# panthuncia/BasicRenderer

Measured on AMD Instinct MI355X. Metric: shaded Mpixels/s @4K (vis-buffer+resolve), higher is better.
Workload: dtype f32; 1 GPU; bistro-class procedural frame, 3840x2160, 1 directional + 256 point lights, 22669824 instanced tris, 2017 instances (2614016 in 150 meshes), LOD DAGs from the library's cluster-LOD builder, relief slope 1.5; pixels_per_gpu=8294400, visible_clusters_rank0=10118, occlusion_culling=True, visible_clusters_phase2_rank0=0, meshlets_tested_rank0=26713, partition=single GPU, frames_in_flight=3

## Files before the change

### basicrenderer_amd/capi.py

```python
import ctypes as C
import os

_HERE = os.path.dirname(os.path.abspath(__file__))
LIB_DIR = os.path.join(_HERE, "lib")

u32, u64, f32, vp = C.c_uint32, C.c_uint64, C.c_float, C.c_void_p


class SceneParams(C.Structure):
    _fields_ = [("preset", u32), ("seed", u32), ("width", u32), ("height", u32), ("numPointLights", u32),
                ("withDirectionalLight", u32), ("lodLevels", u32), ("sizeScale", f32), ("skinnedFraction1024", u32),
                ("materialFeatures", u32), ("cameraStep", u32), ("lodBuilder", u32), ("spotLightEvery", u32), ("detail", f32), ("uniqueTriangleBudget", u32), ("reliefSlope", f32)]


class MeshInput(C.Structure):
    _fields_ = [("positions", vp), ("normals", vp), ("uvs", vp), ("colors", vp), ("vertexCount", C.c_size_t), ("indices", vp), ("indexCount", C.c_size_t),
                ("material", u32), ("reserved", u32 * 3)]


class InstanceInput(C.Structure):
    _fields_ = [("mesh", u32), ("reverseWinding", u32), ("model", (f32 * 4) * 4)]


class ViewInput(C.Structure):
# ... 265 lines not shown
        lib.brmi_scene_export_cache.argtypes = [vp, C.c_char_p]
        lib.brmi_scene_destroy.argtypes = [vp]
        lib.brmi_scene_array.argtypes = [vp, u32, C.POINTER(vp), C.POINTER(u64), C.POINTER(u32)]
        lib.brmi_scene_slab_count.argtypes = [vp]
        lib.brmi_scene_slab_count.restype = u32
        lib.brmi_scene_slab.argtypes = [vp, u32, C.POINTER(vp), C.POINTER(u64)]
        lib.brmi_scene_get_stats.argtypes = [vp, C.POINTER(SceneStats)]
        lib.brmi_scene_camera_at.argtypes = [C.POINTER(SceneParams), C.c_double, C.c_double, vp, vp]
        _scene_lib = lib
    return _scene_lib


BRMI_EXPORTS = ["brmi_abi_version", "brmi_default_config", "brmi_create", "brmi_declare", "brmi_set_scene", "brmi_setup", "brmi_set_band",
                "brmi_update", "brmi_execute", "brmi_execute_split", "brmi_destroy", "brmi_last_error", "brmi_clear_visibility", "brmi_cull",
                "brmi_raster", "brmi_depth_copy", "brmi_build_hzb", "brmi_invalidate_hzb", "brmi_set_history_source", "brmi_gbuffer", "brmi_light_clustering",
                "brmi_shade", "brmi_set_shade_slabs", "brmi_read_counters", "brmi_stage_times", "brmi_set_timed_stages", "brmi_algorithmic_bytes", "brmi_algorithmic_bytes_launched", "brmi_debug_arith", "brmi_debug_arith_in_range", "brmi_debug_read_bin_records", "brmi_debug_wide_triangles", "brmi_debug_lean_clusters", "brmi_debug_read_lean_queue", "brmi_debug_read_held", "brmi_debug_read_draw_list",
                "brmi_streaming_scratch_bytes", "brmi_set_streaming", "brmi_streaming_feedback", "brmi_set_sampler_anisotropy", "brmi_debug_sample_grad",
                "brmi_abi_minor", "brmi_debug_view_bytes", "brmi_set_debug_view", "brmi_debug_view",
                "brmi_set_environment", "brmi_debug_ibl_lookup", "brmi_debug_ibl",
                "brmi_skybox", "brmi_env_convert", "brmi_env_project_sh", "brmi_env_prefilter", "brmi_env_build_bytes", "brmi_debug_env_lookup",
                "brmi_gtao_default_settings", "brmi_gtao_get_layout", "brmi_set_gtao", "brmi_gtao_prefilter", "brmi_gtao_main", "brmi_gtao_denoise",
                "brmi_texmips_bytes", "brmi_texmips_build", "brmi_texmips_build_alpha",
                "brmi_display_default_settings", "brmi_display_get_layout", "brmi_set_display", "brmi_display_exposure", "brmi_display_bloom", "brmi_display_resolve", "brmi_debug_display_bloom_pass", "brmi_debug_display_histogram",
                "brmi_set_shadows", "brmi_shadow_capture", "brmi_debug_shadow"]


def brmi_lib():
    global _brmi_lib
    if _brmi_lib is None:
        import torch
        path = os.environ.get("BRMI_LIB_PATH") or os.path.join(LIB_DIR, "libbrmi.so")
# ... 83 lines not shown
```

### basicrenderer_amd/csrc/brmi_api.hip

```cpp
#include <hip/hip_runtime.h>

#include <algorithm>
#include <cmath>
#include <cstdarg>
#include <cstddef>
#include <cstdio>
#include <cstdlib>
#include <cstring>

#include "brmi_device.h"
#include "brmi_display_math.h"
#include "brmi_internal.h"

namespace brmi {

__global__ void k_debug_arith(const float* a, const float* b, float* outDiv, float* outSqrt, uint32_t* outHalf, uint32_t n) {
    const uint32_t i = blockIdx.x * blockDim.x + threadIdx.x;
    if (i >= n) return;
    outDiv[i] = a[i] / b[i];
    outSqrt[i] = sqrtf(fabsf(a[i]));
    outHalf[i] = f32_to_f16_bits(a[i]);
}

__global__ void k_debug_arith_in_range(const float* a, float* outRcp, float* outSqrt, float* outNorm, uint32_t n) {
// ... 209 lines not shown
        if (cfg->stripeRows == 0u || cfg->stripeRows % 16u || cfg->stripeIndex >= cfg->stripeCount || cfg->bandY0 != 0u || (cfg->bandY1 != 0u && cfg->bandY1 != cfg->height)) return BRMI_ERR_INVALID;
        if (cfg->fullHeight == 0u || cfg->fullHeight % (cfg->stripeRows * cfg->stripeCount) || cfg->height != cfg->fullHeight / cfg->stripeCount) return BRMI_ERR_INVALID;
        if (cfg->dynamicBand) return BRMI_ERR_INVALID;
    }
    if (cfg->dynamicBand && (cfg->bandY0 % 8u || (cfg->bandY1 % 8u && cfg->bandY1 < cfg->height))) return BRMI_ERR_INVALID;
    brmi_pass* p = new brmi_pass();
    p->cfg = *cfg;
    p->totalWords = 1; p->scanBlocks = 1;
    p->forceLevelKernels = tuning("cull_level_kernels", 0) != 0;
    p->packedFlat = tuning("flat_packed", 1) != 0;
    p->flatLevelsMinDraws = (uint32_t)std::max(0l, tuning("flat_levels_min_draws", p->flatLevelsMinDraws));
    p->phase2DirectMax = (uint32_t)std::max(0l, tuning("phase2_direct_max", p->phase2DirectMax));
    p->resolveInlineMode = (int)tuning("resolve_inline", -1);
    p->wideCapacity = (uint32_t)std::min(1l << 20, std::max(0l, tuning("wide_capacity", p->wideCapacity)));
    p->wideMinTriangles = (uint32_t)std::max(0l, tuning("wide_min_triangles", p->wideMinTriangles));
    p->leanMinClusters = (uint32_t)std::max(0l, tuning("lean_min_clusters", p->leanMinClusters));
    if (p->leanMinClusters > cfg->maxVisibleClusters) p->leanMinClusters = 0u;
    p->leanMaxGeneralPct = (uint32_t)std::max(0l, std::min(100l, tuning("lean_max_general_pct", p->leanMaxGeneralPct)));
    p->leanGrid = (uint32_t)std::max(64l, tuning("lean_grid", p->leanGrid));
    p->leanQueue = (uint32_t)std::max(64l, std::min(1l << 24, tuning("lean_queue", p->leanQueue))) & ~63u;
    p->leanWideEntries = (uint32_t)std::max(1l, tuning("lean_wide_entries", p->leanWideEntries));
    p->leanEmitGrid = (uint32_t)std::max(64l, std::min(65536l, tuning("lean_emit_grid", p->leanEmitGrid))) & ~63u;
    p->wideEntries = (uint32_t)std::max(1l, tuning("wide_entries", p->wideEntries));
    p->binMinSlice = (uint32_t)std::max(32l, tuning("bin_min_slice", p->binMinSlice));
    p->binSharedSlice = (uint32_t)std::max(32l, tuning("bin_shared_slice", p->binSharedSlice));
    p->binGrid = (uint32_t)std::min(65535l, std::max(1l, tuning("bin_grid", p->binGrid)));
    p->binOverflowPerStripe = (uint32_t)std::max(0l, tuning("bin_overflow", p->binOverflowPerStripe));
    p->binCapacity = (uint32_t)std::min(65536l, std::max(1l, tuning("bin_capacity", p->binCapacity)));
    if (const long v = tuning("big_tri_area", 0)) p->bigTriArea = p->bigTriAreaAlpha = p->bigTriAreaDense = (int)std::max(1l, v);
    compute_sizes(p);
// ... 786 lines not shown
    out[0] = c[0]; out[1] = c[1]; out[2] = c[2];
    return BRMI_OK;
}

int brmi_debug_lean_clusters(brmi_pass* p, uint32_t out[4]) {
    if (!p || !out || !p->setupDone) return BRMI_ERR_INVALID;
    BRMI_HIP(p, hipDeviceSynchronize());
    uint32_t c = 0u, heads[64 * 32];
    BRMI_HIP(p, hipMemcpy(&c, p->counters() + CNT_GENERAL1, 4, hipMemcpyDeviceToHost));
    BRMI_HIP(p, hipMemcpy(heads, p->counters() + CNT_BIG1, sizeof(heads), hipMemcpyDeviceToHost));
    out[0] = p->leanLastLaunch ? 1u : 0u; out[1] = c; out[2] = out[3] = 0u;
    for (uint32_t s = 0; s < 64u; s++) { out[2] += heads[s * 32u]; out[3] += heads[s * 32u + 1u]; }
    return BRMI_OK;
}

int brmi_debug_read_lean_queue(brmi_pass* p, uint32_t stripe, uint32_t* runs, uint32_t maxRuns, void* entries, uint32_t maxEntries, uint32_t counts[2]) {
    if (!p || !counts || !p->setupDone || stripe >= 64u || p->leanMinClusters == 0u) return BRMI_ERR_INVALID;
    BRMI_HIP(p, hipDeviceSynchronize());
    uint32_t head[2];
    BRMI_HIP(p, hipMemcpy(head, p->counters() + CNT_BIG1 + stripe * 32u, 8, hipMemcpyDeviceToHost));
    const uint32_t cap = p->leanQueue / 64u;
    counts[0] = std::min(head[0], cap); counts[1] = std::min(head[1], cap);
    if (runs) BRMI_HIP(p, hipMemcpy(runs, p->wsPtr<uint8_t>(p->ws.bigRuns) + (size_t)stripe * cap * 8u, (size_t)std::min(maxRuns, counts[1]) * 8u, hipMemcpyDeviceToHost));
    if (entries) BRMI_HIP(p, hipMemcpy(entries, p->wsPtr<uint8_t>(p->ws.bigQueue) + (size_t)stripe * cap * 96u, (size_t)std::min(maxEntries, counts[0]) * 96u, hipMemcpyDeviceToHost));
    return BRMI_OK;
}

int brmi_debug_read_bin_records(brmi_pass* p, void* dst, uint64_t bytes) {
    if (!p || !dst || !p->setupDone) return BRMI_ERR_INVALID;
    BRMI_HIP(p, hipDeviceSynchronize());
// ... 99 lines not shown
```

### basicrenderer_amd/csrc/brmi_device.h

```cpp
#ifndef BRMI_DEVICE_H
#define BRMI_DEVICE_H

#include <hip/hip_runtime.h>
#include <stdint.h>

#include "brmi.h"

#define BRMI_DEV __device__ __forceinline__

namespace brmi {

struct f2 { float x, y; };
struct f3 { float x, y, z; };
struct f4 { float x, y, z, w; };
struct m4 { float m[4][4]; };

BRMI_DEV uint32_t as_u32(float f) { return __float_as_uint(f); }
BRMI_DEV float as_f32(uint32_t u) { return __uint_as_float(u); }

BRMI_DEV f3 operator+(f3 a, f3 b) { return {a.x + b.x, a.y + b.y, a.z + b.z}; }
BRMI_DEV f3 operator-(f3 a, f3 b) { return {a.x - b.x, a.y - b.y, a.z - b.z}; }
BRMI_DEV f3 operator*(f3 a, f3 b) { return {a.x * b.x, a.y * b.y, a.z * b.z}; }
BRMI_DEV f3 operator/(f3 a, f3 b) { return {a.x / b.x, a.y / b.y, a.z / b.z}; }
BRMI_DEV f3 operator*(f3 a, float s) { return {a.x * s, a.y * s, a.z * s}; }
// ... 159 lines not shown
BRMI_DEV uint32_t lane_rank(uint64_t mask) { return __popcll(mask & ((1ull << lane_id()) - 1ull)); }
BRMI_DEV void wave_lds_sync() {
    __builtin_amdgcn_fence(__ATOMIC_RELEASE, "wavefront");
    __builtin_amdgcn_wave_barrier();
    __builtin_amdgcn_fence(__ATOMIC_ACQUIRE, "wavefront");
}
BRMI_DEV m4 load_bone_skin_matrix(const float* skinningMatrices, uint32_t slot, uint32_t joint) {
    const m4 prod = load_m4(skinningMatrices + ((size_t)slot * 64u + joint) * 16u);
    m4 r;
#pragma unroll
    for (int i = 0; i < 4; i++)
#pragma unroll
        for (int j = 0; j < 4; j++) r.m[i][j] = prod.m[j][i];
    return r;
}
BRMI_DEV m4 build_skin_matrix(const float* skinningMatrices, uint32_t slot, const uint32_t* joints, const float* weights) {
    m4 r;
    if (slot == 0xFFFFFFFFu || skinningMatrices == nullptr) {
#pragma unroll
        for (int i = 0; i < 4; i++)
#pragma unroll
            for (int j = 0; j < 4; j++) r.m[i][j] = (i == j) ? 1.0f : 0.0f;
        return r;
    }
#pragma unroll
    for (int k = 0; k < 8; k++) {
        const m4 b = load_bone_skin_matrix(skinningMatrices, slot, joints[k]);
#pragma unroll
        for (int i = 0; i < 4; i++)
#pragma unroll
            for (int j = 0; j < 4; j++) { const float t = weights[k] * b.m[i][j]; r.m[i][j] = (k == 0) ? t : r.m[i][j] + t; }
    }
    return r;
}
BRMI_DEV void load_skin_influences(const uint8_t* jointPtr, const uint8_t* weightPtr, uint32_t joints[8], float weights[8]) {
#pragma unroll
    for (int k = 0; k < 8; k++) { joints[k] = jointPtr ? reinterpret_cast<const uint32_t*>(jointPtr)[k] : 0u; weights[k] = weightPtr ? reinterpret_cast<const float*>(weightPtr)[k] : 0.0f; }
}

BRMI_DEV float ior_to_f0(float ior) { const float s = max2(ior, 1.0f); const float f = (s - 1.0f) / (s + 1.0f); return f * f; }
template <typename T> BRMI_DEV const __attribute__((address_space(4))) T* kconst(const T* p) { return (const __attribute__((address_space(4))) T*)p; }
// ... 30 lines not shown
```

### basicrenderer_amd/csrc/brmi_internal.h

```cpp
#ifndef BRMI_INTERNAL_H
#define BRMI_INTERNAL_H

#include <hip/hip_runtime.h>

#include <string>
#include <vector>

#include "brmi.h"
#include "brmi_device.h"
#include "brmi_scene_tables.h"

#ifndef BRMI_BIN_COUNT_STRIDE
#define BRMI_BIN_COUNT_STRIDE 32
#endif
namespace brmi {

enum CounterIndex : uint32_t {
    CNT_VISIBLE = 3,
    CNT_VISIBLE2,
    CNT_DROPPED_RECORDS,
    CNT_DROPPED_CLUSTERS,
    CNT_INSTANCES_TESTED,
    CNT_INSTANCES_VISIBLE,
    CNT_NODES_VISITED,
// ... 248 lines not shown
    void* res[BRMI_RES_COUNT] = {};
    uint64_t resBytes[BRMI_RES_COUNT] = {};
    uint64_t resNeed[BRMI_RES_COUNT] = {};
    uint32_t tilesX = 0, tilesY = 0;
    uint64_t paddedPixels = 0;
    uint32_t bandY0 = 0, bandY1 = 0;
    brmi::StripeMap stripes{0, 0, 0, 0};
    uint32_t frameHeight() const { return stripes.count > 1u ? stripes.fullHeight : cfg.height; }
    float bandPlaneTop[3] = {0, 0, 0}, bandPlaneBottom[3] = {0, 0, 0};
    uint64_t bandFirstPixel = 0, bandPixelCount = 0;
    uint32_t maxLevels = 1;
    brmi::SceneTables tables;
    bool holdThisFrame = false;
    bool inlineResolve = false;
    bool leanActive = false, leanLastLaunch = false; uint32_t leanRetryIn = 0;
    bool holdEnabled = false;
    uint32_t holdMinClusters = 16384;
    uint32_t lateDirectMax = 128;
    uint32_t holdFloor = 512;
    uint32_t holdStillMax = 8;
    uint32_t holdMaxTexels = 8;
    uint32_t retestMaxTexels = 8;
    uint32_t chainStripLo = 0xFFFFFFFFu, chainStripHi = 0u;
    uint32_t wideCapacity = 16384;
    uint32_t wideEntries = 128;
    uint32_t leanMinClusters = 32768, leanMaxGeneralPct = 40, leanGrid = 24576, leanEmitGrid = 4096, leanWideEntries = 16, leanQueue = 1u << 20;
    uint32_t wideMinTriangles = 4;
    std::vector<float> sliceStartHost; float sliceKey[3] = {0, 0, 0}; uint32_t sliceKeyN[2] = {0, 0};
    brmi::HostFeedback feedback;
    uint32_t phase2DirectMax = 128;
// ... 120 lines not shown
```

### basicrenderer_amd/csrc/brmi_raster.hip

```cpp
#include <algorithm>

#include "brmi_device.h"
#include "brmi_internal.h"
#include "brmi_texture.h"

namespace brmi {

struct BinRecord {
    uint32_t clusterIndex, triAndFlags;
    int32_t  minX, rectWidth, rowStart;
    float    sb0, sb1, dx_b0, dx_b1, dy_b0, dy_b1, d0, d1, d2;
    uint32_t pad0, pad1;
};
static_assert(sizeof(BinRecord) == 64, "one cache line");
struct AlphaRecord { AlphaTri tri; uint32_t materialDataIndex, pad[2]; };
static_assert(sizeof(AlphaRecord) == 48, "AlphaRecord layout");
constexpr int BIN_W = 256, BIN_ROWS = 16;
constexpr int BIN_W_SHIFT = 8, BIN_ROWS_SHIFT = 4;
constexpr uint32_t BIN_COUNT_STRIDE = BRMI_BIN_COUNT_STRIDE;
constexpr int BIN_WINDOW = 256;
constexpr int COOP_ENTRIES = 64;
#ifndef BRMI_COOP_ENTRIES_TABLE
#define BRMI_COOP_ENTRIES_TABLE 512
#endif
// ... 187 lines not shown
    bin_store(a, unorm, r, ar, strip, band, atomicAdd(&a.binCounts[(size_t)(band * a.binsX + strip) * BIN_COUNT_STRIDE], 1u));
}

#ifndef BRMI_RASTER_WAVES
#define BRMI_RASTER_WAVES 3
#endif
#ifndef BRMI_RASTER_ALPHA_WAVES
#define BRMI_RASTER_ALPHA_WAVES 2
#endif
#ifndef BRMI_RASTER_SPLIT_FIRST
#define BRMI_RASTER_SPLIT_FIRST 2u
#endif
#ifndef BRMI_RASTER_LEAN_WAVES
#define BRMI_RASTER_LEAN_WAVES 6
#endif
template <bool ALPHA, bool LEAN = false>
__global__ void __launch_bounds__(64, LEAN ? BRMI_RASTER_LEAN_WAVES : (ALPHA ? BRMI_RASTER_ALPHA_WAVES : BRMI_RASTER_WAVES)) k_raster(RasterArgs a) {
    static_assert(!(ALPHA && LEAN), "the lean form has no alpha test");
    __shared__ float sx[BRMI_MESHLET_MAX_VERTS], sy[BRMI_MESHLET_MAX_VERTS], sd[BRMI_MESHLET_MAX_VERTS];
    __shared__ float siw[ALPHA ? BRMI_MESHLET_MAX_VERTS : 1], su[ALPHA ? BRMI_MESHLET_MAX_VERTS : 1], sv[ALPHA ? BRMI_MESHLET_MAX_VERTS : 1];
    __shared__ float tpA[ALPHA ? 9 : 1][64];
    __shared__ float unormT[ALPHA ? 256 : 1];
    if (ALPHA) { for (uint32_t i = threadIdx.x; i < 256u; i += 64u) unormT[i] = (float)i / 255.0f; __syncthreads(); }
    extern __shared__ uint32_t binBase[];
    __shared__ float tpF[9][64];
    __shared__ int tpI[4][64];
    __shared__ uint32_t rowOff[65];
    const brmi_scene_buffers& sc = a.sc;
    const uint32_t lane = threadIdx.x;
    const uint32_t first = (uint32_t)__builtin_amdgcn_readfirstlane((int)(a.firstCounter == 0xFFFFFFFFu ? 0u : a.counters[a.firstCounter]));
    const uint32_t count = (uint32_t)__builtin_amdgcn_readfirstlane((int)a.counters[a.countCounter]);
    if (a.countFeedback && blockIdx.x == 0u && lane == 0u) __hip_atomic_store(a.countFeedback, count, __ATOMIC_RELAXED, __HIP_MEMORY_SCOPE_SYSTEM);
    const GlobalSink gsink{a.vis, a.tilesX};
// ... 34 lines not shown
        const bool reverseWinding = ((cs.counts >> 24) & 1u) != 0u;
        const brmi_view_raster_info ri = load_uniform(&sc.viewRasterInfo[cs.viewId]);
        const float visWidth = (float)(ri.scissorMaxX - ri.scissorMinX), visHeight = (float)(ri.scissorMaxY - ri.scissorMinY);
        const float sMinXf = (float)ri.scissorMinX, sMinYf = (float)ri.scissorMinY;
        const auto oc = kconst(a.objConst + (size_t)cs.perObjectIndex * OBJ_CONST_FLOATS);
        m4 mvp;
#pragma unroll
        for (int i = 0; i < 4; i++)
#pragma unroll
            for (int j = 0; j < 4; j++) mvp.m[i][j] = oc[i * 4 + j];
        const f4 modelViewZ{oc[32], oc[33], oc[34], oc[35]};
        const uint8_t* posBase = cs.posBase;
        const uint8_t* triBase = cs.triBase;
        uint32_t pi0[2] = {0u, 0u}, pi1[2] = {0u, 0u}, pi2[2] = {0u, 0u};
#pragma unroll
        for (uint32_t k = 0; k < 2u; k++) {
            const uint32_t t = passLo + k * 64u + lane;
            if (passLo + k * 64u < passHi && t < triCount) { pi0[k] = triBase[t * 3u]; pi1[k] = triBase[t * 3u + 1u]; pi2[k] = triBase[t * 3u + 2u]; }
        }
        const bool skinVerts = !LEAN && (cs.counts & (BRMI_CS_SKINNED | BRMI_CS_JOINTS)) == (BRMI_CS_SKINNED | BRMI_CS_JOINTS);
        const uint32_t skinSlot = skinVerts ? sc.perMeshInstance[cs.instanceIndex].skinningInstanceSlot : 0xFFFFFFFFu;
        const bool alphaCluster = ALPHA && (cs.counts & BRMI_CS_ALPHA) != 0u;
        ClusterUv cu{nullptr, nullptr};
        AlphaMaterial amat{};
        if (alphaCluster) { cu = a.clusterUv[clusterIndex]; amat = a.alphaMats[cs.materialDataIndex]; }

        if (!toGeneral)
        for (uint32_t v = lane; v < vertCount; v += 64) {
            f3 lp{0.0f, 0.0f, 0.0f};
            if (posFormat == BRMI_POSITION_FORMAT_FLOAT3) {
                const float* pp = reinterpret_cast<const float*>(posBase + v * 12u);
                lp = f3{pp[0], pp[1], pp[2]};
            }
            if (skinVerts) {
                uint32_t joints[8]; float weights[8];
                load_skin_influences(cs.nrmBase + cs.jointDelta + v * 32u, (cs.counts & BRMI_CS_WEIGHTS) ? cs.nrmBase + cs.weightDelta + v * 32u : nullptr, joints, weights);
                lp = xyz(mul_point(lp, build_skin_matrix(sc.skinningMatrices, skinSlot, joints, weights)));
            }
            const f4 lp4{lp.x, lp.y, lp.z, 1.0f};
            const f4 clip = mul_vm(lp4, mvp);
            const float viewZ = dot4(lp4, modelViewZ);
            const float invW = 1.0f / clip.w;
            const float ndcx = clip.x * invW, ndcy = clip.y * invW;
            sx[v] = (ndcx + 1.0f) * 0.5f * visWidth + sMinXf;
            sy[v] = (1.0f - ndcy) * 0.5f * visHeight + sMinYf;
            sd[v] = -viewZ;
            if (alphaCluster) { const f2 uv = decode_uv(cu, v); siw[v] = invW; su[v] = uv.x; sv[v] = uv.y; }
        }
        wave_lds_sync();

        for (uint32_t waveBase = passLo; waveBase < passHi && !toGeneral; waveBase += 64) {
            const uint32_t t = waveBase + lane;
            bool active = t < triCount;
            float d0 = 0, d1 = 0, d2 = 0, row_b0 = 0, row_b1 = 0, dx_b0 = 0, dx_b1 = 0, dy_b0 = 0, dy_b1 = 0;
            int minX = 0, minY = 0, maxX = -1, maxY = -1;
            AlphaRecord arec{};
            if (active) {
                const uint32_t pk = (waveBase - passLo) >> 6;
                uint32_t i0 = pk ? pi0[1] : pi0[0], i1 = pk ? pi1[1] : pi1[0], i2 = pk ? pi2[1] : pi2[0];
                if (reverseWinding) { const uint32_t tmp = i1; i1 = i2; i2 = tmp; }
                if (alphaCluster) { arec.tri = AlphaTri{siw[i0], siw[i1], siw[i2], f2{su[i0], sv[i0]}, f2{su[i1], sv[i1]}, f2{su[i2], sv[i2]}}; arec.materialDataIndex = cs.materialDataIndex; }
                const float s0x = sx[i0], s0y = sy[i0], s1x = sx[i1], s1y = sy[i1], s2x = sx[i2], s2y = sy[i2];
                d0 = sd[i0]; d1 = sd[i1]; d2 = sd[i2];
                if (d0 <= 0.0f || d1 <= 0.0f || d2 <= 0.0f) active = false;
                const float e01x = s1x - s0x, e01y = s1y - s0y, e02x = s2x - s0x, e02y = s2y - s0y;
                const float twiceArea = e01x * e02y - e01y * e02x;
                if (twiceArea >= 0.0f) active = false;
                if (active) {
                    const float invTwiceArea = -1.0f / twiceArea;
                    const float bbMinX = min2(min2(s0x, s1x), s2x), bbMinY = min2(min2(s0y, s1y), s2y);
                    const float bbMaxX = max2(max2(s0x, s1x), s2x), bbMaxY = max2(max2(s0y, s1y), s2y);
                    minX = to_int_sat(floorf(bbMinX)); minY = to_int_sat(floorf(bbMinY));
                    maxX = to_int_sat(floorf(bbMaxX)); maxY = to_int_sat(floorf(bbMaxY));
                    minX = max(minX, (int)ri.scissorMinX); minY = max(minY, (int)ri.scissorMinY);
// ... 259 lines not shown
                                          f2{__shfl(arec.tri.uv1.x, src), __shfl(arec.tri.uv1.y, src)}, f2{__shfl(arec.tri.uv2.x, src), __shfl(arec.tri.uv2.y, src)}};
                    c_arec.materialDataIndex = cs.materialDataIndex;
                }
                float sb0 = c_sb0, sb1 = c_sb1;
                int py = c_yLo;
                for (int band = c_band0 + (int)lane; band <= c_band1; band += 64) {
                    if (!owns_band(band)) continue;
                    const int start = max(band << BIN_ROWS_SHIFT, c_yLo);
                    for (; py < start; py++) { sb0 += c_dy0; sb1 += c_dy1; }
                    const int n = min(((band + 1) << BIN_ROWS_SHIFT), c_yHi + 1) - start;
                    BinRecord r;
                    r.clusterIndex = clusterIndex; r.triAndFlags = c_flags | ((uint32_t)n << 16);
                    r.minX = c_minX; r.rectWidth = c_w; r.rowStart = striped ? (int)stripe_vrow(a.stripes, (uint32_t)start) : start;
                    const uint32_t vb = vband(band);
                    r.sb0 = sb0; r.sb1 = sb1; r.dx_b0 = c_dx0; r.dx_b1 = c_dx1; r.dy_b0 = c_dy0; r.dy_b1 = c_dy1; r.d0 = c_d0; r.d1 = c_d1; r.d2 = c_d2; r.pad0 = 0; r.pad1 = alphaCluster ? 1u : 0u;
                    for (int st0 = c_strip0; st0 <= c_strip1; st0 += 8) {
                        uint32_t slots[8];
#pragma unroll
                        for (int k = 0; k < 8; k++) slots[k] = (st0 + k <= c_strip1) ? atomicAdd(&a.binCounts[(size_t)(vb * a.binsX + (uint32_t)(st0 + k)) * BIN_COUNT_STRIDE], 1u) : 0u;
#pragma unroll
                        for (int k = 0; k < 8; k++) if (st0 + k <= c_strip1) bin_store(a, unormT, r, c_arec, (uint32_t)(st0 + k), vb, slots[k]);
                    }
                }
            }
        }
        if (LEAN && toGeneral && lane == 0u) a.generalList[atomicAdd(&a.counters[a.generalCounter], 1u)] = clusterIndex;
        wave_lds_sync();
    }
    if (ALPHA && rqTail != rqHead) rq_drain(rqTail - rqHead);
}

__global__ void __launch_bounds__(64) k_raster_emit(RasterArgs a) {
    extern __shared__ uint32_t binBase[];
    const uint32_t lane = threadIdx.x;
    const uint32_t stripe = blockIdx.x & 63u;
    const uint32_t nRuns = min((uint32_t)__builtin_amdgcn_readfirstlane((int)a.counters[a.bigCounter + stripe * 32u + 1u]), a.bigCapacity);
    const AlphaRecord noAlpha{};
    for (uint32_t run = blockIdx.x >> 6; run < nRuns; run += gridDim.x >> 6) {
        const uint2 rd = load_uniform(&a.bigRuns[(size_t)stripe * a.bigCapacity + run]);
        const bool have = lane < rd.y;
        WideTri w{};
        if (have) w = a.bigQueue[(size_t)stripe * a.bigCapacity + rd.x + lane];
        w.pad[0] = w.pad[1] = w.pad[2] = 0u;
        const int nStrips = w.strip1 - w.strip0 + 1;
        int entries = have ? (w.band1 - w.band0 + 1) * nStrips : 0;
// ... 605 lines not shown
    a.tableCells = std::max<uint32_t>(BIN_WINDOW, std::min<uint32_t>(BIN_TABLE_MAX, (p->binsX * p->binsY + 63u) & ~63u));
    a.binAlpha = p->wsPtr<AlphaRecord>(p->ws.binAlpha); a.overflowAlpha = p->wsPtr<AlphaRecord>(p->ws.overflowAlpha);
    a.clusterUv = p->wsPtr<ClusterUv>(p->ws.clusterUv);
    a.alphaMats = p->wsPtr<AlphaMaterial>(p->ws.alphaMats);
    if (p->tables.hasAlphaTest && p->scene.materialCount > (1u << 20)) return fail(p, BRMI_ERR_INVALID, "brmi_raster: %u materials in a scene with alpha-tested ones (at most %u)", p->scene.materialCount, 1u << 20);
    if (p->tables.hasAlphaTest) if (int rc = ensure_frame_constants(p, ctx, s)) return rc;
    const uint32_t hint2 = phase == 2 ? p->feedback.last(FB_PLACED2, 0xFFFFFFFFu) : 0xFFFFFFFFu;
    auto pow2_at_least = [](uint32_t v) { uint32_t r = 1; while (r < v && r < (1u << 30)) r <<= 1; return r; };
    const bool sized2 = hint2 < 128u;
    const dim3 bgrid(phase == 2 ? (sized2 ? std::max(16u, std::min(256u, pow2_at_least(hint2 * 2u))) : std::min(p->binGrid, 256u)) : p->binGrid);
    const bool direct2 = phase == 2 && !p->tables.hasAlphaTest && p->feedback.dev(FB_PLACED2) && hint2 <= p->phase2DirectMax && p->phase2DirectMax != 0u;
    if (direct2) a.bigTriArea = a.bigTriAreaAlpha = a.bigTriAreaDense = 0x3FFFFFFF;
    constexpr uint32_t grid2 = 2048;
    const dim3 rgrid(phase == 2 ? std::min(p->rasterGrid, sized2 ? std::max(128u, std::min(grid2, pow2_at_least(hint2 * 16u))) : grid2) : p->rasterGrid);
    const dim3 ogrid(phase == 2 && sized2 ? std::max(2u, std::min(129u, hint2 / 4u + 2u)) : 129u);
    auto chain = [&](auto alpha, const RasterArgs& ra, bool rasterLaunched, dim3 rg, dim3 og, dim3 bg, bool direct) {
        constexpr bool ALPHA = decltype(alpha)::value;
        if (!rasterLaunched) hipLaunchKernelGGL(k_raster<ALPHA>, rg, dim3(64), ra.tableCells * 4u, s, ra);
        if (direct) return;
        if (wideOn) hipLaunchKernelGGL(k_raster_wide<ALPHA>, wgrid, dim3(64), 0, s, ra);
        if (!ALPHA && p->binsX * p->binsY > 4096u) hipLaunchKernelGGL((k_raster_overflow<false, 1024>), dim3((og.x - 1u + 3u) / 4u + 1u), dim3(1024), 0, s, ra);
        else hipLaunchKernelGGL(k_raster_overflow<ALPHA>, og, dim3(256), 0, s, ra);
        hipLaunchKernelGGL(k_raster_bins<ALPHA>, bg, dim3(BRMI_BIN_THREADS), 0, s, ra);
    };
    if (p->tables.hasAlphaTest) chain(std::true_type{}, a, false, rgrid, ogrid, bgrid, direct2);
    else {
        uint32_t* const leanFeedback = (phase == 1 && p->leanMinClusters != 0u && p->stripes.count <= 1u) ? p->feedback.dev(FB_LEAN_COUNT) : nullptr;
        bool lean = false;
        if (leanFeedback) {
            const uint32_t lastCount = p->feedback.last(FB_LEAN_COUNT, 0u), lastGeneral = p->feedback.last(FB_GENERAL_COUNT, 0u);
            if (p->leanActive) {
                if (lastCount < p->leanMinClusters) p->leanActive = false;
                else if ((uint64_t)lastGeneral * 100u > (uint64_t)lastCount * p->leanMaxGeneralPct) { p->leanActive = false; p->leanRetryIn = 64u; }
            } else if (p->leanRetryIn != 0u) p->leanRetryIn--;
            else if (lastCount >= p->leanMinClusters) { p->leanActive = true; p->feedback.store(FB_GENERAL_COUNT, 0u); }
            lean = p->leanActive;
            a.countFeedback = leanFeedback;
        }
        if (phase == 1) p->leanLastLaunch = lean;
        if (lean) {
            a.generalList = p->wsPtr<uint32_t>(p->ws.generalList); a.generalCounter = CNT_GENERAL1; a.generalFeedback = p->feedback.dev(FB_GENERAL_COUNT);
            a.bigQueue = p->wsPtr<WideTri>(p->ws.bigQueue); a.bigRuns = p->wsPtr<uint2>(p->ws.bigRuns); a.bigCapacity = p->leanQueue / 64u; a.bigCounter = CNT_BIG1;
            hipLaunchKernelGGL((k_raster<false, true>), dim3(p->leanGrid), dim3(64), 0, s, a);
            hipLaunchKernelGGL(k_raster_emit, dim3(p->leanEmitGrid), dim3(64), a.tableCells * 4u, s, a);
            RasterArgs g = a;
            g.drawList = a.generalList; g.firstCounter = 0xFFFFFFFFu; g.countCounter = CNT_GENERAL1; g.countFeedback = p->feedback.dev(FB_GENERAL_COUNT);
            const dim3 ggrid(std::min(p->rasterGrid, std::max(128u, pow2_at_least(std::min(p->feedback.last(FB_GENERAL_COUNT, 0u), 1u << 20) * 16u))));
            hipLaunchKernelGGL(k_raster<false>, ggrid, dim3(64), g.tableCells * 4u, s, g);
        }
        chain(std::false_type{}, a, lean, rgrid, ogrid, bgrid, direct2);
    }
    BRMI_LAUNCH_CHECK(p, "k_raster");
    if (hold) {
        if (int rc = launch_hzb(p, ctx, s, ChainBuild::InRaster)) return rc;
        const uint32_t lastLate = p->feedback.last(FB_LATE, 0u), lastHeld = p->feedback.last(FB_HELD, 0xFFFFFFFFu);
        RetestArgs r;
        r.held = p->wsPtr<HeldRecord>(p->ws.heldRecords); r.boxes = p->wsPtr<MeshletBox>(p->ws.meshletBoxes); r.objConst = a.objConst; r.viewRasterInfo = p->scene.viewRasterInfo;
        r.hzb = p->hzbDesc(); r.visW = a.visW; r.visH = a.visH; r.capacity = p->cfg.maxVisibleClusters; r.maxTexels = p->retestMaxTexels; r.bandY0 = p->bandY0; r.bandY1 = p->bandY1;
        r.counters = p->counters(); r.lateList = p->wsPtr<uint32_t>(p->ws.lateList); r.heldFeedback = p->feedback.dev(FB_HELD);
        const uint32_t tgrid = std::max(16u, std::min(4096u, pow2_at_least(std::min(lastHeld, p->cfg.maxVisibleClusters) / 256u + 1u)));
        hipLaunchKernelGGL(k_retest_held, dim3(tgrid), dim3(256), 0, s, r);
        RasterArgs l = a;
        l.drawList = r.lateList; l.countCounter = CNT_LATE1; l.countFeedback = p->feedback.dev(FB_LATE);
// ... 22 lines not shown
```

### basicrenderer_amd/renderer.py

```python
import ctypes as C

import numpy as np

from . import capi


class BrmiError(RuntimeError):
    pass


def detile(flat, width, height, tile=8):
    tx, ty = (width + tile - 1) // tile, (height + tile - 1) // tile
    rest = flat.shape[1:]
    a = flat.reshape((ty, tx, tile, tile) + rest)
    a = np.transpose(a, (0, 3, 1, 2) + tuple(range(4, 4 + len(rest)))).reshape((ty * tile, tx * tile) + rest)
    return np.ascontiguousarray(a[:height, :width])


def tile(img, tile=8):
    height, width = img.shape[:2]
    tx, ty = (width + tile - 1) // tile, (height + tile - 1) // tile
    rest = img.shape[2:]
    pad = np.zeros((ty * tile, tx * tile) + rest, dtype=img.dtype)
    pad[:height, :width] = img
# ... 189 lines not shown

    def draw_list(self):
        nd, nh, nb = capi.u32(), capi.u32(), capi.u32()
        self._check(self.lib.brmi_debug_read_draw_list(self._h, None, 0, C.byref(nd), None, 0, C.byref(nh), C.byref(nb)), "brmi_debug_read_draw_list")
        if nd.value > self.cfg.maxVisibleClusters or nh.value > self.cfg.maxVisibleClusters:
            raise BrmiError(f"draw list of {nd.value} / held list of {nh.value} entries in buffers of {self.cfg.maxVisibleClusters}")
        draw, boxes = np.zeros(max(1, nd.value), dtype=np.uint32), np.zeros(max(1, nh.value), dtype=np.uint32)
        self._check(self.lib.brmi_debug_read_draw_list(self._h, draw.ctypes.data_as(C.POINTER(capi.u32)), len(draw), C.byref(nd), boxes.ctypes.data_as(C.POINTER(capi.u32)), len(boxes), C.byref(nh), C.byref(nb)), "brmi_debug_read_draw_list")
        return draw[: nd.value], boxes[: nh.value], int(nb.value)

    def lean_clusters(self):
        out = (capi.u32 * 4)()
        self._check(self.lib.brmi_debug_lean_clusters(self._h, out), "brmi_debug_lean_clusters")
        return tuple(int(v) for v in out)

    def wide_triangles(self):
        out = (capi.u32 * 3)()
        self._check(self.lib.brmi_debug_wide_triangles(self._h, out), "brmi_debug_wide_triangles")
        return tuple(int(x) for x in out)

    def algorithmic_bytes_launched(self):
        per = (capi.u64 * len(capi.STAGE_NAMES))()
        total = capi.u64()
        self._check(self.lib.brmi_algorithmic_bytes_launched(self._h, per, C.byref(total)), "brmi_algorithmic_bytes_launched")
        return dict(zip(capi.STAGE_NAMES, [int(x) for x in per])), int(total.value)

    def _img(self, rid, dtype, comps=1):
        self.torch.cuda.synchronize(self.device)
        raw = self.res[capi.RES[rid]].cpu().numpy()
        a = raw.view(dtype)
# ... 463 lines not shown
```

### include/brmi.h

```cpp
#ifndef BRMI_H
#define BRMI_H

#include <stdint.h>
#include "brmi_types.h"

#ifdef __cplusplus
extern "C" {
#endif

#define BRMI_ABI_VERSION 1u
#define BRMI_ABI_MINOR 1u

typedef enum brmi_status {
    BRMI_OK            = 0,
    BRMI_ERR_INVALID   = -1,
    BRMI_ERR_HIP       = -2,
    BRMI_ERR_CAPACITY  = -3,
    BRMI_ERR_STATE     = -4
} brmi_status;

typedef struct brmi_pass brmi_pass;
typedef void* brmi_stream;

typedef struct brmi_config {
// ... 273 lines not shown
int brmi_light_clustering(brmi_pass* pass, brmi_stream stream);
int brmi_shade(brmi_pass* pass, brmi_stream stream);
typedef void (*brmi_slab_fn)(void* user, uint32_t row0, uint32_t row1, brmi_stream stream);
int brmi_set_shade_slabs(brmi_pass* pass, uint32_t slabs, brmi_slab_fn fn, void* user);

int brmi_read_counters(brmi_pass* pass, brmi_counters* out, brmi_stream stream);
int brmi_stage_times(brmi_pass* pass, float* msOut );
int brmi_set_timed_stages(brmi_pass* pass, uint32_t stageMask);
int brmi_algorithmic_bytes(brmi_pass* pass, uint64_t* perStage , uint64_t* total);
int brmi_algorithmic_bytes_launched(brmi_pass* pass, uint64_t* perStage , uint64_t* total);

int brmi_debug_arith(const float* a, const float* b, float* outDiv, float* outSqrt, uint32_t* outHalfBits, uint32_t n, brmi_stream stream);

int brmi_debug_wide_triangles(brmi_pass* pass, uint32_t out[3]);
int brmi_debug_lean_clusters(brmi_pass* pass, uint32_t out[4]);
int brmi_debug_read_lean_queue(brmi_pass* pass, uint32_t stripe, uint32_t* runs, uint32_t maxRuns, void* entries, uint32_t maxEntries, uint32_t counts[2]);

int brmi_debug_read_held(brmi_pass* pass, uint32_t* held, uint32_t heldCapacity, uint32_t* heldCount, uint32_t* late, uint32_t lateCapacity, uint32_t* lateCount);
int brmi_debug_read_draw_list(brmi_pass* pass, uint32_t* draw, uint32_t drawCapacity, uint32_t* drawCount, uint32_t* heldBoxes, uint32_t heldCapacity, uint32_t* heldCount, uint32_t* boxCount);

int brmi_debug_read_bin_records(brmi_pass* pass, void* dst, uint64_t bytes);

int brmi_debug_arith_in_range(const float* a, float* outRcp, float* outSqrt, float* outRsqrt, uint32_t n, brmi_stream stream);


int brmi_debug_sample_grad(const brmi_scene_buffers* scene, const uint32_t* maxAnisotropy , uint32_t textureIndex,
                           uint32_t samplerIndex, uint32_t uniformBinding, const float* uv, const float* ddx, const float* ddy, float* outRGBA,
                           uint32_t n, brmi_stream stream);

int brmi_debug_ibl_lookup(const brmi_environment_buffers* env, uint32_t cubemapIndex, const float* directions, const float* lods, float* outRGBA, uint32_t n,
// ... 23 lines not shown
```

Before: 18230 Mpixels/s.

## Add register-slim opaque raster kernel variant capped at 52 VGPRs

Adds a slim instantiation of the opaque direct rasteriser that caps VGPRs at 52 to raise occupancy. It drops the prefetched triangle-index registers in favour of reloading indices at use, limits skinning loads in flight with scheduling barriers, and halves the bin-slot atomic batch. By default it is chosen only when no alpha-tested materials exist and the context uses two streams. Fewer registers may trade latency hiding per wave and extra index loads for more resident waves.

```diff
diff --git a/basicrenderer_amd/capi.py b/basicrenderer_amd/capi.py
--- a/basicrenderer_amd/capi.py
+++ b/basicrenderer_amd/capi.py
@@ -303,7 +303,7 @@
 BRMI_EXPORTS = ["brmi_abi_version", "brmi_default_config", "brmi_create", "brmi_declare", "brmi_set_scene", "brmi_setup", "brmi_set_band",
                 "brmi_update", "brmi_execute", "brmi_execute_split", "brmi_destroy", "brmi_last_error", "brmi_clear_visibility", "brmi_cull",
                 "brmi_raster", "brmi_depth_copy", "brmi_build_hzb", "brmi_invalidate_hzb", "brmi_set_history_source", "brmi_gbuffer", "brmi_light_clustering",
-                "brmi_shade", "brmi_set_shade_slabs", "brmi_read_counters", "brmi_stage_times", "brmi_set_timed_stages", "brmi_algorithmic_bytes", "brmi_algorithmic_bytes_launched", "brmi_debug_arith", "brmi_debug_arith_in_range", "brmi_debug_read_bin_records", "brmi_debug_wide_triangles", "brmi_debug_lean_clusters", "brmi_debug_read_lean_queue", "brmi_debug_read_held", "brmi_debug_read_draw_list",
+                "brmi_shade", "brmi_set_shade_slabs", "brmi_read_counters", "brmi_stage_times", "brmi_set_timed_stages", "brmi_algorithmic_bytes", "brmi_algorithmic_bytes_launched", "brmi_debug_arith", "brmi_debug_arith_in_range", "brmi_debug_read_bin_records", "brmi_debug_wide_triangles", "brmi_debug_lean_clusters", "brmi_debug_raster_shape", "brmi_debug_read_lean_queue", "brmi_debug_read_held", "brmi_debug_read_draw_list",
                 "brmi_streaming_scratch_bytes", "brmi_set_streaming", "brmi_streaming_feedback", "brmi_set_sampler_anisotropy", "brmi_debug_sample_grad",
                 "brmi_abi_minor", "brmi_debug_view_bytes", "brmi_set_debug_view", "brmi_debug_view",
                 "brmi_set_environment", "brmi_debug_ibl_lookup", "brmi_debug_ibl",
diff --git a/basicrenderer_amd/csrc/brmi_api.hip b/basicrenderer_amd/csrc/brmi_api.hip
--- a/basicrenderer_amd/csrc/brmi_api.hip
+++ b/basicrenderer_amd/csrc/brmi_api.hip
@@ -247,6 +247,7 @@
     p->resolveInlineMode = (int)tuning("resolve_inline", -1);
     p->wideCapacity = (uint32_t)std::min(1l << 20, std::max(0l, tuning("wide_capacity", p->wideCapacity)));
     p->wideMinTriangles = (uint32_t)std::max(0l, tuning("wide_min_triangles", p->wideMinTriangles));
+    p->rasterSlim = (int)std::max(-1l, std::min(1l, tuning("raster_slim", -1)));
     p->leanMinClusters = (uint32_t)std::max(0l, tuning("lean_min_clusters", p->leanMinClusters));
     if (p->leanMinClusters > cfg->maxVisibleClusters) p->leanMinClusters = 0u;
     p->leanMaxGeneralPct = (uint32_t)std::max(0l, std::min(100l, tuning("lean_max_general_pct", p->leanMaxGeneralPct)));
@@ -1063,6 +1064,12 @@
     return BRMI_OK;
 }
 
+int brmi_debug_raster_shape(brmi_pass* p, uint32_t* slim) {
+    if (!p || !slim || !p->setupDone) return BRMI_ERR_INVALID;
+    *slim = p->slimLastLaunch ? 1u : 0u;
+    return BRMI_OK;
+}
+
 int brmi_debug_read_lean_queue(brmi_pass* p, uint32_t stripe, uint32_t* runs, uint32_t maxRuns, void* entries, uint32_t maxEntries, uint32_t counts[2]) {
     if (!p || !counts || !p->setupDone || stripe >= 64u || p->leanMinClusters == 0u) return BRMI_ERR_INVALID;
     BRMI_HIP(p, hipDeviceSynchronize());
diff --git a/basicrenderer_amd/csrc/brmi_device.h b/basicrenderer_amd/csrc/brmi_device.h
--- a/basicrenderer_amd/csrc/brmi_device.h
+++ b/basicrenderer_amd/csrc/brmi_device.h
@@ -197,6 +197,7 @@
         for (int j = 0; j < 4; j++) r.m[i][j] = prod.m[j][i];
     return r;
 }
+template <int IN_FLIGHT = 8>
 BRMI_DEV m4 build_skin_matrix(const float* skinningMatrices, uint32_t slot, const uint32_t* joints, const float* weights) {
     m4 r;
     if (slot == 0xFFFFFFFFu || skinningMatrices == nullptr) {
@@ -208,6 +209,7 @@
     }
 #pragma unroll
     for (int k = 0; k < 8; k++) {
+        if (IN_FLIGHT < 8 && k != 0 && k % IN_FLIGHT == 0) __builtin_amdgcn_sched_barrier(0);
         const m4 b = load_bone_skin_matrix(skinningMatrices, slot, joints[k]);
 #pragma unroll
         for (int i = 0; i < 4; i++)
diff --git a/basicrenderer_amd/csrc/brmi_internal.h b/basicrenderer_amd/csrc/brmi_internal.h
--- a/basicrenderer_amd/csrc/brmi_internal.h
+++ b/basicrenderer_amd/csrc/brmi_internal.h
@@ -286,6 +286,7 @@
     bool holdThisFrame = false;
     bool inlineResolve = false;
     bool leanActive = false, leanLastLaunch = false; uint32_t leanRetryIn = 0;
+    int rasterSlim = -1; bool slimLastLaunch = false;
     bool holdEnabled = false;
     uint32_t holdMinClusters = 16384;
     uint32_t lateDirectMax = 128;
diff --git a/basicrenderer_amd/csrc/brmi_raster.hip b/basicrenderer_amd/csrc/brmi_raster.hip
--- a/basicrenderer_amd/csrc/brmi_raster.hip
+++ b/basicrenderer_amd/csrc/brmi_raster.hip
@@ -225,9 +225,10 @@
 #ifndef BRMI_RASTER_LEAN_WAVES
 #define BRMI_RASTER_LEAN_WAVES 6
 #endif
-template <bool ALPHA, bool LEAN = false>
-__global__ void __launch_bounds__(64, LEAN ? BRMI_RASTER_LEAN_WAVES : (ALPHA ? BRMI_RASTER_ALPHA_WAVES : BRMI_RASTER_WAVES)) k_raster(RasterArgs a) {
+template <bool ALPHA, bool LEAN, bool SLIM>
+BRMI_DEV void raster_clusters(RasterArgs a) {
     static_assert(!(ALPHA && LEAN), "the lean form has no alpha test");
+    static_assert(!SLIM || (!ALPHA && !LEAN), "the slim shape is the opaque direct rasteriser's");
     __shared__ float sx[BRMI_MESHLET_MAX_VERTS], sy[BRMI_MESHLET_MAX_VERTS], sd[BRMI_MESHLET_MAX_VERTS];
     __shared__ float siw[ALPHA ? BRMI_MESHLET_MAX_VERTS : 1], su[ALPHA ? BRMI_MESHLET_MAX_VERTS : 1], sv[ALPHA ? BRMI_MESHLET_MAX_VERTS : 1];
     __shared__ float tpA[ALPHA ? 9 : 1][64];
@@ -292,7 +293,7 @@
         const uint8_t* triBase = cs.triBase;
         uint32_t pi0[2] = {0u, 0u}, pi1[2] = {0u, 0u}, pi2[2] = {0u, 0u};
 #pragma unroll
-        for (uint32_t k = 0; k < 2u; k++) {
+        for (uint32_t k = 0; k < (SLIM ? 0u : 2u); k++) {
             const uint32_t t = passLo + k * 64u + lane;
             if (passLo + k * 64u < passHi && t < triCount) { pi0[k] = triBase[t * 3u]; pi1[k] = triBase[t * 3u + 1u]; pi2[k] = triBase[t * 3u + 2u]; }
         }
@@ -303,8 +304,10 @@
         AlphaMaterial amat{};
         if (alphaCluster) { cu = a.clusterUv[clusterIndex]; amat = a.alphaMats[cs.materialDataIndex]; }
 
+        uint32_t vlane = lane;
+        if (SLIM) asm volatile("" : "+v"(vlane));
         if (!toGeneral)
-        for (uint32_t v = lane; v < vertCount; v += 64) {
+        for (uint32_t v = vlane; v < vertCount; v += 64) {
             f3 lp{0.0f, 0.0f, 0.0f};
             if (posFormat == BRMI_POSITION_FORMAT_FLOAT3) {
                 const float* pp = reinterpret_cast<const float*>(posBase + v * 12u);
@@ -313,7 +316,7 @@
             if (skinVerts) {
                 uint32_t joints[8]; float weights[8];
                 load_skin_influences(cs.nrmBase + cs.jointDelta + v * 32u, (cs.counts & BRMI_CS_WEIGHTS) ? cs.nrmBase + cs.weightDelta + v * 32u : nullptr, joints, weights);
-                lp = xyz(mul_point(lp, build_skin_matrix(sc.skinningMatrices, skinSlot, joints, weights)));
+                lp = xyz(mul_point(lp, build_skin_matrix<SLIM ? 2 : 8>(sc.skinningMatrices, skinSlot, joints, weights)));
             }
             const f4 lp4{lp.x, lp.y, lp.z, 1.0f};
             const f4 clip = mul_vm(lp4, mvp);
@@ -336,6 +339,7 @@
             if (active) {
                 const uint32_t pk = (waveBase - passLo) >> 6;
                 uint32_t i0 = pk ? pi0[1] : pi0[0], i1 = pk ? pi1[1] : pi1[0], i2 = pk ? pi2[1] : pi2[0];
+                if (SLIM) { i0 = triBase[t * 3u]; i1 = triBase[t * 3u + 1u]; i2 = triBase[t * 3u + 2u]; }
                 if (reverseWinding) { const uint32_t tmp = i1; i1 = i2; i2 = tmp; }
                 if (alphaCluster) { arec.tri = AlphaTri{siw[i0], siw[i1], siw[i2], f2{su[i0], sv[i0]}, f2{su[i1], sv[i1]}, f2{su[i2], sv[i2]}}; arec.materialDataIndex = cs.materialDataIndex; }
                 const float s0x = sx[i0], s0y = sy[i0], s1x = sx[i1], s1y = sy[i1], s2x = sx[i2], s2y = sy[i2];
@@ -625,12 +629,13 @@
                     r.minX = c_minX; r.rectWidth = c_w; r.rowStart = striped ? (int)stripe_vrow(a.stripes, (uint32_t)start) : start;
                     const uint32_t vb = vband(band);
                     r.sb0 = sb0; r.sb1 = sb1; r.dx_b0 = c_dx0; r.dx_b1 = c_dx1; r.dy_b0 = c_dy0; r.dy_b1 = c_dy1; r.d0 = c_d0; r.d1 = c_d1; r.d2 = c_d2; r.pad0 = 0; r.pad1 = alphaCluster ? 1u : 0u;
-                    for (int st0 = c_strip0; st0 <= c_strip1; st0 += 8) {
-                        uint32_t slots[8];
-#pragma unroll
-                        for (int k = 0; k < 8; k++) slots[k] = (st0 + k <= c_strip1) ? atomicAdd(&a.binCounts[(size_t)(vb * a.binsX + (uint32_t)(st0 + k)) * BIN_COUNT_STRIDE], 1u) : 0u;
-#pragma unroll
-                        for (int k = 0; k < 8; k++) if (st0 + k <= c_strip1) bin_store(a, unormT, r, c_arec, (uint32_t)(st0 + k), vb, slots[k]);
+                    constexpr int SLOTS = SLIM ? 4 : 8;
+                    for (int st0 = c_strip0; st0 <= c_strip1; st0 += SLOTS) {
+                        uint32_t slots[SLOTS];
+#pragma unroll
+                        for (int k = 0; k < SLOTS; k++) slots[k] = (st0 + k <= c_strip1) ? atomicAdd(&a.binCounts[(size_t)(vb * a.binsX + (uint32_t)(st0 + k)) * BIN_COUNT_STRIDE], 1u) : 0u;
+#pragma unroll
+                        for (int k = 0; k < SLOTS; k++) if (st0 + k <= c_strip1) bin_store(a, unormT, r, c_arec, (uint32_t)(st0 + k), vb, slots[k]);
                     }
                 }
             }
@@ -640,6 +645,9 @@
     }
     if (ALPHA && rqTail != rqHead) rq_drain(rqTail - rqHead);
 }
+template <bool ALPHA, bool LEAN = false>
+__global__ void __launch_bounds__(64, LEAN ? BRMI_RASTER_LEAN_WAVES : (ALPHA ? BRMI_RASTER_ALPHA_WAVES : BRMI_RASTER_WAVES)) k_raster(RasterArgs a) { raster_clusters<ALPHA, LEAN, false>(a); }
+__global__ void __launch_bounds__(64) __attribute__((amdgpu_num_vgpr(52))) k_raster_slim(RasterArgs a) { raster_clusters<false, false, true>(a); }
 
 __global__ void __launch_bounds__(64) k_raster_emit(RasterArgs a) {
     extern __shared__ uint32_t binBase[];
@@ -1275,9 +1283,14 @@
     constexpr uint32_t grid2 = 2048;
     const dim3 rgrid(phase == 2 ? std::min(p->rasterGrid, sized2 ? std::max(128u, std::min(grid2, pow2_at_least(hint2 * 16u))) : grid2) : p->rasterGrid);
     const dim3 ogrid(phase == 2 && sized2 ? std::max(2u, std::min(129u, hint2 / 4u + 2u)) : 129u);
+    const bool slim = !p->tables.hasAlphaTest && (p->rasterSlim < 0 ? ctx.twoStreams : p->rasterSlim != 0);
+    if (phase == 1) p->slimLastLaunch = false;
     auto chain = [&](auto alpha, const RasterArgs& ra, bool rasterLaunched, dim3 rg, dim3 og, dim3 bg, bool direct) {
         constexpr bool ALPHA = decltype(alpha)::value;
-        if (!rasterLaunched) hipLaunchKernelGGL(k_raster<ALPHA>, rg, dim3(64), ra.tableCells * 4u, s, ra);
+        if (!rasterLaunched) {
+            if (!ALPHA && slim) { hipLaunchKernelGGL(k_raster_slim, rg, dim3(64), ra.tableCells * 4u, s, ra); if (phase == 1) p->slimLastLaunch = true; }
+            else hipLaunchKernelGGL(k_raster<ALPHA>, rg, dim3(64), ra.tableCells * 4u, s, ra);
+        }
         if (direct) return;
         if (wideOn) hipLaunchKernelGGL(k_raster_wide<ALPHA>, wgrid, dim3(64), 0, s, ra);
         if (!ALPHA && p->binsX * p->binsY > 4096u) hipLaunchKernelGGL((k_raster_overflow<false, 1024>), dim3((og.x - 1u + 3u) / 4u + 1u), dim3(1024), 0, s, ra);
@@ -1307,7 +1320,8 @@
             RasterArgs g = a;
             g.drawList = a.generalList; g.firstCounter = 0xFFFFFFFFu; g.countCounter = CNT_GENERAL1; g.countFeedback = p->feedback.dev(FB_GENERAL_COUNT);
             const dim3 ggrid(std::min(p->rasterGrid, std::max(128u, pow2_at_least(std::min(p->feedback.last(FB_GENERAL_COUNT, 0u), 1u << 20) * 16u))));
-            hipLaunchKernelGGL(k_raster<false>, ggrid, dim3(64), g.tableCells * 4u, s, g);
+            if (slim) { hipLaunchKernelGGL(k_raster_slim, ggrid, dim3(64), g.tableCells * 4u, s, g); if (phase == 1) p->slimLastLaunch = true; }
+            else hipLaunchKernelGGL(k_raster<false>, ggrid, dim3(64), g.tableCells * 4u, s, g);
         }
         chain(std::false_type{}, a, lean, rgrid, ogrid, bgrid, direct2);
     }
diff --git a/basicrenderer_amd/renderer.py b/basicrenderer_amd/renderer.py
--- a/basicrenderer_amd/renderer.py
+++ b/basicrenderer_amd/renderer.py
@@ -227,6 +227,11 @@
         self._check(self.lib.brmi_debug_lean_clusters(self._h, out), "brmi_debug_lean_clusters")
         return tuple(int(v) for v in out)
 
+    def raster_shape(self):
+        out = capi.u32(0)
+        self._check(self.lib.brmi_debug_raster_shape(self._h, C.byref(out)), "brmi_debug_raster_shape")
+        return int(out.value)
+
     def wide_triangles(self):
         out = (capi.u32 * 3)()
         self._check(self.lib.brmi_debug_wide_triangles(self._h, out), "brmi_debug_wide_triangles")
diff --git a/include/brmi.h b/include/brmi.h
--- a/include/brmi.h
+++ b/include/brmi.h
@@ -311,6 +311,7 @@
 
 int brmi_debug_wide_triangles(brmi_pass* pass, uint32_t out[3]);
 int brmi_debug_lean_clusters(brmi_pass* pass, uint32_t out[4]);
+int brmi_debug_raster_shape(brmi_pass* pass, uint32_t* slim);
 int brmi_debug_read_lean_queue(brmi_pass* pass, uint32_t stripe, uint32_t* runs, uint32_t maxRuns, void* entries, uint32_t maxEntries, uint32_t counts[2]);
 
 int brmi_debug_read_held(brmi_pass* pass, uint32_t* held, uint32_t heldCapacity, uint32_t* heldCount, uint32_t* late, uint32_t lateCapacity, uint32_t* lateCount);
```

New measurement: 18490 Mpixels/s (median of 6 runs). 1.4% higher.
